# FluxML/Flux3D.jl

Measured on AMD Instinct MI355X. Metric: chamfer_point_pairs_per_sec, higher is better.
Workload: dtype f32

## Files before the change

flux3d.jl_amd/csrc/chamfer.hip:

```cpp
#include <atomic>
#include <cmath>
#include <cstdlib>
#include <mutex>

#include "fx3d_common.h"

using namespace fx3d;

#ifdef FX3D_PROBE
__device__ unsigned long long g_probe[4096 * 16];
#define FX3D_PROBE_MARK(k)                                                                   \
    do {                                                                                     \
        if (threadIdx.x == 0 && blockIdx.x < 4096) {                                         \
            g_probe[blockIdx.x * 16 + (k)] = __builtin_readcyclecounter();                   \
            if ((k) == 0) g_probe[blockIdx.x * 16 + 13] = wall_clock64();                    \
            if ((k) == 12) g_probe[blockIdx.x * 16 + 14] = wall_clock64();                   \
        }                                                                                    \
    } while (0)
__device__ unsigned long long g_probe2[256 * 16];
#define FX3D_PROBE_MARK2(k) do { if (threadIdx.x == 0 && blockIdx.x < 256) g_probe2[blockIdx.x * 16 + (k)] = __builtin_readcyclecounter(); } while (0)
__device__ unsigned long long g_probe3[16 * 16 * 8];
#define FX3D_PROBE_MARKW(k) do { if ((threadIdx.x & 63) == 0 && blockIdx.x < 16) g_probe3[(blockIdx.x * 16 + (threadIdx.x >> 6)) * 8 + (k)] = __builtin_readcyclecounter(); } while (0)
#else
#define FX3D_PROBE_MARK(k) do { } while (0)
// ... 311 lines not shown
__device__ __forceinline__ float vmin(float a, float b) {
    float r;
    asm("v_min_f32 %0, %1, %2" : "=v"(r) : "v"(a), "v"(b));
    return r;
}

__device__ __forceinline__ void split2h(float v, _Float16 &h, _Float16 &l) {
    h = (_Float16)v;
    l = (_Float16)(v - (float)h);
}

constexpr float kBetaC = 0x1.1p-18f;
constexpr float kBandB1 = 1.0f + 18.0f * kBetaC + 0x1p-20f;
constexpr float kBandA = 22.3f * kBetaC + 0x1p-19f;
__device__ __forceinline__ void make_pieces(float cx, float cy, float cz, h8 &p0, h8 &p1) {
    _Float16 hx, lx, hy, ly, hz, lz, n1, n2, n3;
    split2h(cx, hx, lx); split2h(cy, hy, ly); split2h(cz, hz, lz);
    const float n0 = ((cx * cx) + (cy * cy)) + (cz * cz);
    const float n = n0 + kBetaC * n0;
    n1 = (_Float16)n;
    const float r1 = n - (float)n1;
    n2 = (_Float16)r1;
    n3 = (_Float16)(r1 - (float)n2);
    const _Float16 z = (_Float16)0.0f;
    p0 = h8{hx, hx, lx, hy, hy, ly, hz, hz};
    p1 = h8{lz, n1, n2, n3, lx, ly, lz, z};
}

template <bool WANT_IDX, bool SPLITFUSE = false, bool PRUNE = false>
__global__ __launch_bounds__(kHThreads, 4) void nn1_f16_kernel(Nn1Params p) {
    extern __shared__ __attribute__((aligned(16))) float lds[];
    __shared__ __attribute__((aligned(16))) float red[4 * 4 * (kHThreads / 64) + 16];
    __shared__ int nfar[2];
    __shared__ unsigned short farlist[kHFarCap];
    constexpr int QB = (kHThreads / 64) * 32;

    const int L = blockIdx.x;
    const int per_cloud = p.tiles * p.nsplit;
    const bool by_xcd = 2 * p.B >= 8;
    const int slot = by_xcd ? L >> 3 : L;
    const int c = by_xcd ? (slot / per_cloud) * 8 + (L & 7) : slot / per_cloud;
    const int tile = (slot % per_cloud) / p.nsplit;
    const int split = (slot % per_cloud) % p.nsplit;
    if (c >= 2 * p.B) return;
    const int dir = c >= p.B ? 1 : 0;
    const int b = dir ? c - p.B : c;
    const int NQ = dir ? p.M : p.N;
    const int NC = dir ? p.N : p.M;
    if (tile >= (dir ? p.tiles_y : p.tiles_x)) return;
    if ((long long)split * p.chunk >= NC) return;
    const int ctail = (p.tail > 0 && p.nsplit == 1 && NC > p.chunk && NC - p.chunk <= p.tail) ? NC - p.chunk : 0;
    const int NCm = NC - ctail;
    const float *__restrict__ qb = (dir ? p.y : p.x) + (size_t)b * NQ * 3;
    const float *__restrict__ cb = (dir ? p.x : p.y) + (size_t)b * NC * 3;
    int32_t *idx_out = dir ? p.idx_y : p.idx_x;
    float *dmin_out = dir ? p.dmin_y : p.dmin_x;

    const int tid = threadIdx.x, lane = tid & 63;
    const int wv = __builtin_amdgcn_readfirstlane(tid >> 6);
    const int jq = lane & 31, hh = lane >> 5;
    const int CH = p.chunk;
    const int tpb = dir ? p.tpb_y : p.tpb;
    h8 *imgp = reinterpret_cast<h8 *>(lds);
    float4 *imgf = reinterpret_cast<float4 *>(lds);
    unsigned long long *wres = reinterpret_cast<unsigned long long *>(lds + 8 * (CH + 64));
    unsigned short *witems = reinterpret_cast<unsigned short *>(wres + (kHThreads / 64) * 32);
    float *wq = reinterpret_cast<float *>(witems + (kHThreads / 64) * kHItemCap);
    unsigned long long *qres = wres + wv * 32;
    unsigned short *items = witems + wv * kHItemCap;
    float *qtab = wq + wv * 96;
    const bool vec = (reinterpret_cast<uintptr_t>(cb) & 15) == 0;
    const bool one_shot = NCm <= CH;
    if (tid == 0) { nfar[0] = 0; nfar[1] = 0; }
    float qpre[3];
    {
        const int q0i = (tile * tpb) * QB + wv * 32 + jq;
        const int qc0 = q0i < NQ ? q0i : NQ - 1;
#pragma unroll
        for (int d = 0; d < 3; ++d) qpre[d] = qb[(size_t)qc0 * 3 + d];
    }
    if constexpr (PRUNE) {
        unsigned int *zc = reinterpret_cast<unsigned int *>(wres);
        for (int i = tid; i < 1040 + 16 * 256; i += kHThreads) zc[i] = 0u;
        int *gb = reinterpret_cast<int *>(wq + (kHThreads / 64) * 96) + 64 * 8;
        for (int i = tid; i < kHGroupsMax * 8; i += kHThreads) gb[i] = (i & 4) ? (int)0x80000000 : 0x7fffffff;
    }
    FX3D_PROBE_MARK(0);

    const bool own_chunk_only = p.nsplit > 1 && (long long)split * CH + (long long)p.nsplit * CH >= NCm;
    const int s_lo = own_chunk_only ? split * CH : 0;
    const int SN = own_chunk_only ? (NCm - s_lo < CH ? NCm - s_lo : CH) : NC;
    const float *__restrict__ sb = cb + (size_t)s_lo * 3;
    const bool parked = one_shot || own_chunk_only;
    float mu[3], cinf = 0.0f, varmax = 0.0f;
    float bxlo[3] = {0.f, 0.f, 0.f}, bxhi[3] = {0.f, 0.f, 0.f};
    bool allfin = true;
    {
        float mn[3] = {INFINITY, INFINITY, INFINITY}, mx[3] = {-INFINITY, -INFINITY, -INFINITY}, sm3[3] = {0.f, 0.f, 0.f};
        float sqt = 0.0f;
        const float pil[3] = {sb[0], sb[1], sb[2]};
        const int nsweep = (SN + kHThreads - 1) / kHThreads;
        for (int i0 = 0; i0 < nsweep; i0 += 4) {
            P3 v[4];
#pragma unroll
            for (int e = 0; e < 4; ++e) {
                const int pt = (i0 + e) * kHThreads + tid;
                v[e] = *reinterpret_cast<const P3 *>(sb + (size_t)(pt < SN ? pt : SN - 1) * 3);
            }
#pragma unroll
            for (int e = 0; e < 4; ++e) {
                const int pt = (i0 + e) * kHThreads + tid;
                mn[0] = fminf(mn[0], v[e].x); mx[0] = fmaxf(mx[0], v[e].x);
                mn[1] = fminf(mn[1], v[e].y); mx[1] = fmaxf(mx[1], v[e].y);
                mn[2] = fminf(mn[2], v[e].z); mx[2] = fmaxf(mx[2], v[e].z);
                if (pt < SN) {
                    sm3[0] = sm3[0] + v[e].x; sm3[1] = sm3[1] + v[e].y; sm3[2] = sm3[2] + v[e].z;
                    if (parked) imgf[((pt >> 5) * 2) * 32 + (pt & 31)] = float4{v[e].x, v[e].y, v[e].z, 0.0f};
                }
                if (((i0 + e) & 3) == (wv & 3) && pt < SN) {
                    sqt = __builtin_fmaf(v[e].x - pil[0], v[e].x - pil[0], sqt); sqt = __builtin_fmaf(v[e].y - pil[1], v[e].y - pil[1], sqt);
                    sqt = __builtin_fmaf(v[e].z - pil[2], v[e].z - pil[2], sqt);
                }
            }
        }
        FX3D_PROBE_MARK(5);
        {
            float4 lo4, hi4, st4;
            lo4.x = wave_min_l63(mn[0]); lo4.y = wave_min_l63(mn[1]); lo4.z = wave_min_l63(mn[2]); lo4.w = 0.0f;
            hi4.x = wave_max_l63(mx[0]); hi4.y = wave_max_l63(mx[1]); hi4.z = wave_max_l63(mx[2]); hi4.w = 0.0f;
            st4.x = wave_sum_l63(sm3[0]); st4.y = wave_sum_l63(sm3[1]); st4.z = wave_sum_l63(sm3[2]); st4.w = wave_sum_l63(sqt);
            if (lane == 63) {
                float4 *r4 = reinterpret_cast<float4 *>(red);
                r4[wv * 4] = lo4; r4[wv * 4 + 1] = hi4; r4[wv * 4 + 2] = st4;
            }
        }
        FX3D_PROBE_MARK(9);
        __syncthreads();
        FX3D_PROBE_MARK(10);
        static_assert(kHThreads / 64 == 16, "the cross-wave reduction below: one wave's row of 16 lanes, one lane per wave");
        if (wv == 0) {
            const float4 *r4 = reinterpret_cast<const float4 *>(red);
            const int w = lane & 15;
            float4 lo4 = r4[w * 4], hi4 = r4[w * 4 + 1], st4 = r4[w * 4 + 2];
#define NN1_ROW_MIN(v) v = fkey_inv(row_mm_key<false>(fkey(v)));
#define NN1_ROW_MAX(v) v = fkey_inv(row_mm_key<true>(fkey(v)));
#define NN1_ROW_SUM(v) v = v + dpp_mov<0xB1>(v); v = v + dpp_mov<0x4E>(v); v = v + dpp_mov<0x141>(v); v = v + dpp_mov<0x140>(v);
            NN1_ROW_MIN(lo4.x) NN1_ROW_MIN(lo4.y) NN1_ROW_MIN(lo4.z)
            NN1_ROW_MAX(hi4.x) NN1_ROW_MAX(hi4.y) NN1_ROW_MAX(hi4.z)
            NN1_ROW_SUM(st4.x) NN1_ROW_SUM(st4.y) NN1_ROW_SUM(st4.z) NN1_ROW_SUM(st4.w)
#undef NN1_ROW_MIN
#undef NN1_ROW_MAX
#undef NN1_ROW_SUM
            const float lo3[3] = {lo4.x, lo4.y, lo4.z}, hi3[3] = {hi4.x, hi4.y, hi4.z}, st3[3] = {st4.x, st4.y, st4.z};
            float m3[3], ci = 0.0f, vm = st4.w / fmaxf(0.25f * (float)SN, 1.0f);
            bool fin = true;
#pragma unroll
            for (int d = 0; d < 3; ++d) {
                const float lo = lo3[d], hi = hi3[d], st = st3[d];
                m3[d] = fminf(fmaxf(st / (float)SN, lo), hi);
                const float off = st / (float)SN - pil[d];
                vm = vm - off * off;
                ci = fmaxf(ci, fmaxf(hi - m3[d], m3[d] - lo));
                fin = fin && fabsf(st) < INFINITY;
            }
            if (lane == 0) {
                float4 *o4 = reinterpret_cast<float4 *>(red) + 4 * (kHThreads / 64);
                o4[0] = float4{m3[0], m3[1], m3[2], ci * 1.000001f};
                o4[1] = float4{vm, fin ? 1.0f : 0.0f, 0.0f, 0.0f};
                if (PRUNE) { o4[2] = float4{lo3[0], lo3[1], lo3[2], 0.0f}; o4[3] = float4{hi3[0], hi3[1], hi3[2], 0.0f}; }
            }
        }
        __syncthreads();
        {
            const float4 *o4 = reinterpret_cast<const float4 *>(red) + 4 * (kHThreads / 64);
            const float4 a = o4[0], b2 = o4[1];
            mu[0] = a.x; mu[1] = a.y; mu[2] = a.z; cinf = a.w;
            varmax = b2.x; allfin = b2.y != 0.0f;
            if (PRUNE) {
                const float4 l4 = o4[2], h4 = o4[3];
                bxlo[0] = l4.x; bxlo[1] = l4.y; bxlo[2] = l4.z; bxhi[0] = h4.x; bxhi[1] = h4.y; bxhi[2] = h4.z;
            }
        }
    }
    float rng = cinf;
    if (allfin && cinf < 1.0e16f && 3.0f * cinf * cinf > kRobustGate * varmax) {
        const float4 r = robust_range3<kHThreads, false>(sb, SN, parked, imgf, red, mu[0], mu[1], mu[2], cinf);
        mu[0] = r.x; mu[1] = r.y; mu[2] = r.z; rng = r.w;
    }
    const bool sane = allfin && cinf < 1.0e16f;
    float sc = 1.0f;
    if (sane && rng > 1.0e-30f) {
        int e;
        (void)frexpf(rng, &e);
        sc = ldexpf(1.0f, 7 - e);
    }
    auto uni = [](float v) { return __builtin_bit_cast(float, __builtin_amdgcn_readfirstlane(__builtin_bit_cast(int, v))); };
    mu[0] = uni(mu[0]); mu[1] = uni(mu[1]); mu[2] = uni(mu[2]); sc = uni(sc); rng = uni(rng); cinf = uni(cinf);
    const bool has_far = sane && rng < cinf;
    int fslot = 0;
    auto pieces = [&](float x, float y, float z, int pt, h8 &p0, h8 &p1) {
        const float sx = (x - mu[0]) * sc, sy = (y - mu[1]) * sc, sz = (z - mu[2]) * sc;
        if (!has_far) { make_pieces(sx, sy, sz, p0, p1); return; }
        const bool far = !(fmaxf(fmaxf(fabsf(sx), fabsf(sy)), fabsf(sz)) < 128.0f);
        make_pieces(far ? 0.f : sx, far ? 0.f : sy, far ? 0.f : sz, p0, p1);
        if (far) {
            p1[7] = (_Float16)kPadF16;
            const int f = atomicAdd(&nfar[fslot], 1);
            if (f < kHFarCap) farlist[f] = (unsigned short)pt;
        }
    };

    [[maybe_unused]] float4 *cs = nullptr, *qsw = nullptr;
    [[maybe_unused]] bool sorted_c = false;
    [[maybe_unused]] int qwlen = 0;
    [[maybe_unused]] float4 *boxes = nullptr;
    if constexpr (PRUNE) {
        cs = p.pscr + (size_t)blockIdx.x * p.pscr_stride;
        qsw = cs + kHChunkMax;
        boxes = reinterpret_cast<float4 *>(wq + (kHThreads / 64) * 96);
        unsigned int *ccnt = reinterpret_cast<unsigned int *>(wres);
        unsigned int *qtot = ccnt + 520;
        unsigned int *qwh = qtot + 520;
        const bool last_t = tile == (dir ? p.tiles_y : p.tiles_x) - 1;
        const int qw0 = tile * tpb * QB;
        const int qw1 = last_t || qw0 + tpb * QB > NQ ? NQ : qw0 + tpb * QB;
        qwlen = qw1 - qw0;
        const int cnt = NCm;
        const bool do_sort = sane && cnt >= 512;
        const bool sorted_q = do_sort && NQ <= 4 * kHThreads;
        P3 qv[4];
        if (sorted_q) {
#pragma unroll
            for (int e = 0; e < 4; ++e) {
                const int qp = 256 * wv + 64 * e + lane;
                qv[e] = *reinterpret_cast<const P3 *>(qb + (size_t)(qp < NQ ? qp : NQ - 1) * 3);
            }
        }
        FX3D_PROBE_MARK2(0);
        int *gbox = reinterpret_cast<int *>(boxes + 64 * 2);
        auto group_box = [&](int wrow, float x, float y, float z) {
            int *g = gbox + (wrow >> 5) * 8;
            atomicMin(g + 0, fkey((x - mu[0]) * sc)); atomicMin(g + 1, fkey((y - mu[1]) * sc)); atomicMin(g + 2, fkey((z - mu[2]) * sc));
            atomicMax(g + 4, fkey((x - mu[0]) * sc)); atomicMax(g + 5, fkey((y - mu[1]) * sc)); atomicMax(g + 6, fkey((z - mu[2]) * sc));
        };
        if (do_sort) {
            float4 cv[4];
#pragma unroll
            for (int e = 0; e < 4; ++e) {
                const int pt = e * kHThreads + tid;
                cv[e] = float4{0.f, 0.f, 0.f, 0.f};
                if (pt < cnt) cv[e] = imgf[((pt >> 5) * 2) * 32 + (pt & 31)];
            }
            FX3D_PROBE_MARK2(1);
            float inv[3], off[3], cfl[3], cfh[3];
#pragma unroll
            for (int d = 0; d < 3; ++d) {
                const float fr = has_far ? 0.125f * rng : 128.0f / sc;
                const float flo = fmaxf(bxlo[d], mu[d] - fr), fhi = fminf(bxhi[d], mu[d] + fr);
                inv[d] = fhi > flo ? 8.0f / (fhi - flo) : 0.0f;
                off[d] = -flo * inv[d];
                cfl[d] = flo; cfh[d] = fhi;
            }
            auto cell = [&](float x, float y, float z) -> unsigned int {
                const unsigned int ux = (unsigned int)(int)fminf(fmaxf(__builtin_fmaf(x, inv[0], off[0]), 0.0f), 7.0f);
                const unsigned int uy = (unsigned int)(int)fminf(fmaxf(__builtin_fmaf(y, inv[1], off[1]), 0.0f), 7.0f);
                const unsigned int uz = (unsigned int)(int)fminf(fmaxf(__builtin_fmaf(z, inv[2], off[2]), 0.0f), 7.0f);
                return ux | (uy << 3) | (uz << 6);
            };

            unsigned int ccr[4], qcr[4];
            auto count_cells = [&](bool valid, unsigned int t, auto &&add) -> unsigned int {
                unsigned int rank = 0u;
                bool mine = valid;
                const unsigned int tn = (unsigned int)__builtin_amdgcn_update_dpp((int)~t, (int)t, 0x111, 0xF, 0xF, false);
                if (__builtin_popcountll(__ballot(valid && t == tn)) >= 8) {
                    unsigned long long rem = __ballot(valid);
                    for (int it = 0; it < 12 && rem; ++it) {
                        const unsigned int t0 = (unsigned int)__builtin_amdgcn_readlane((int)t, __builtin_ctzll(rem));
                        const unsigned long long grp = __ballot(mine && t == t0);
                        rem &= ~grp;
                        if (__builtin_popcountll(grp) < 4) continue;
                        unsigned int base = 0u;
                        if ((int)lane == __builtin_ctzll(grp)) base = add(t0, (unsigned int)__builtin_popcountll(grp));
                        base = (unsigned int)__builtin_amdgcn_readlane((int)base, __builtin_ctzll(grp));
                        if (mine && t == t0) {
                            rank = base + __builtin_amdgcn_mbcnt_hi((unsigned int)(grp >> 32), __builtin_amdgcn_mbcnt_lo((unsigned int)grp, 0u));
                            mine = false;
                        }
                    }
                }
                if (mine) rank = add(t, 1u);
                return rank;
            };
#pragma unroll
            for (int e = 0; e < 4; ++e) {
                const int pt = e * kHThreads + tid;
                const unsigned int t = pt < cnt ? cell(cv[e].x, cv[e].y, cv[e].z) : 0u;
                ccr[e] = (t << 16) | count_cells(pt < cnt, t, [&](unsigned int c, unsigned int n) { return atomicAdd(&ccnt[c], n); });
            }
            int *qbb = reinterpret_cast<int *>(boxes + 64 * 2 + kHGroupsMax * 2 - 2);
            if (sorted_q) {
                int kl[3] = {0x7fffffff, 0x7fffffff, 0x7fffffff}, kh[3] = {(int)0x80000000, (int)0x80000000, (int)0x80000000};
#pragma unroll
                for (int e = 0; e < 4; ++e) {
                    const int qp = 256 * wv + 64 * e + lane;
                    if (qp < NQ) {
                        const int k3[3] = {fkey(qv[e].x), fkey(qv[e].y), fkey(qv[e].z)};
#pragma unroll
                        for (int d = 0; d < 3; ++d) { kl[d] = kl[d] < k3[d] ? kl[d] : k3[d]; kh[d] = kh[d] > k3[d] ? kh[d] : k3[d]; }
                    }
                }
#pragma unroll
                for (int d = 0; d < 3; ++d) {
                    int a = row_mm_key<false>(kl[d]), b2 = row_mm_key<true>(kh[d]);
                    a = imm<false>(a, dpp_keepi<0x142, 0xA>(a)); a = imm<false>(a, dpp_keepi<0x143, 0xC>(a));
                    b2 = imm<true>(b2, dpp_keepi<0x142, 0xA>(b2)); b2 = imm<true>(b2, dpp_keepi<0x143, 0xC>(b2));
                    if (lane == 63) { atomicMin(qbb + d, a); atomicMax(qbb + 4 + d, b2); }
                }
            }
            FX3D_PROBE_MARK2(2);
            __syncthreads();
            FX3D_PROBE_MARK2(3);
            float qinv[3] = {0.f, 0.f, 0.f}, qoff[3] = {0.f, 0.f, 0.f};
            if (sorted_q) {
                const float ext = fmaxf(fmaxf(cfh[0] - cfl[0], cfh[1] - cfl[1]), cfh[2] - cfl[2]);
#pragma unroll
                for (int d = 0; d < 3; ++d) {
                    const float ql = fkey_inv(qbb[d]), qh = fkey_inv(qbb[4 + d]);
                    const float grow = qh - ql > 4.0f * ext ? 0.25f * ext : ext;
                    const float lo = fmaxf(ql, cfl[d] - grow), hi = fminf(qh, cfh[d] + grow);
                    qinv[d] = hi > lo && hi - lo < INFINITY ? 8.0f / (hi - lo) : 0.0f;
                    qoff[d] = qinv[d] != 0.0f ? -lo * qinv[d] : 0.0f;
                }
            }
            auto qcell = [&](float x, float y, float z) -> unsigned int {
                const unsigned int ux = (unsigned int)(int)fminf(fmaxf(__builtin_fmaf(x, qinv[0], qoff[0]), 0.0f), 7.0f);
                const unsigned int uy = (unsigned int)(int)fminf(fmaxf(__builtin_fmaf(y, qinv[1], qoff[1]), 0.0f), 7.0f);
                const unsigned int uz = (unsigned int)(int)fminf(fmaxf(__builtin_fmaf(z, qinv[2], qoff[2]), 0.0f), 7.0f);
                return ux | (uy << 3) | (uz << 6);
            };
            auto curve_scan = [&](unsigned int *a) {
                unsigned int tc[8];
                {
                    const uint4 h = *reinterpret_cast<const uint4 *>(kHilbertCell + 8 * lane);
                    tc[0] = h.x & 0xffffu; tc[1] = h.x >> 16; tc[2] = h.y & 0xffffu; tc[3] = h.y >> 16;
                    tc[4] = h.z & 0xffffu; tc[5] = h.z >> 16; tc[6] = h.w & 0xffffu; tc[7] = h.w >> 16;
                }
                unsigned int c8[8], tot = 0u;
#pragma unroll
                for (int k = 0; k < 8; ++k) { c8[k] = a[tc[k]]; tot += c8[k]; }
                unsigned int inc = tot;
#pragma unroll
                for (int o = 1; o < 64; o <<= 1) {
                    const unsigned int v = __shfl_up(inc, o, 64);
                    if (lane >= o) inc += v;
                }
                unsigned int run = inc - tot;
#pragma unroll
                for (int k = 0; k < 8; ++k) { a[tc[k]] = run; run += c8[k]; }
            };
            if (wv == 0) curve_scan(ccnt);
            if (sorted_q) {
#pragma unroll
                for (int e = 0; e < 4; ++e) {
                    const int qp = 256 * wv + 64 * e + lane;
                    const unsigned int t = qp < NQ ? qcell(qv[e].x, qv[e].y, qv[e].z) : 0u;
                    qcr[e] = (t << 16) | count_cells(qp < NQ, t, [&](unsigned int c, unsigned int n) {
                                 const unsigned int sh = 16u * (c & 1u);
                                 const unsigned int old = atomicAdd(&qwh[wv * 256 + (c >> 1)], n << sh);
                                 atomicAdd(&qtot[c], n);
                                 return (old >> sh) & 0xffffu;
                             });
                }
            }
            FX3D_PROBE_MARK2(4);
            __syncthreads();
            FX3D_PROBE_MARK2(5);
#pragma unroll
            for (int e = 0; e < 4; ++e) {
                const int pt = e * kHThreads + tid;
                if (pt < cnt) {
                    const int pos = (int)(ccnt[ccr[e] >> 16] + (ccr[e] & 0xffffu));
                    imgf[((pos >> 5) * 2) * 32 + (pos & 31)] = float4{cv[e].x, cv[e].y, cv[e].z, __builtin_bit_cast(float, pt)};
                }
            }
            sorted_c = true;
            if (sorted_q) {
                if (wv == 1) {
                    curve_scan(qtot);
                } else if (wv >= 2 && wv < 6) {
                    const int w2 = tid - 128;
                    unsigned int run = 0u;
#pragma unroll
                    for (int w = 0; w < 16; ++w) {
                        const unsigned int v = qwh[w * 256 + w2];
                        qwh[w * 256 + w2] = run;
                        run += v;
                    }
                }
            }
            FX3D_PROBE_MARK2(6);
            __syncthreads();
            FX3D_PROBE_MARK2(7);
            if (sorted_q) {
#pragma unroll
                for (int e = 0; e < 4; ++e) {
                    const int qp = 256 * wv + 64 * e + lane;
                    if (qp < NQ) {
                        const unsigned int t = qcr[e] >> 16;
                        const int rank = (int)(qtot[t] + ((qwh[wv * 256 + (t >> 1)] >> (16u * (t & 1u))) & 0xffffu) + (qcr[e] & 0xffffu));
                        if (rank >= qw0 && rank < qw1) {
                            qsw[rank - qw0] = float4{qv[e].x, qv[e].y, qv[e].z, __builtin_bit_cast(float, qp)};
                            group_box(rank - qw0, qv[e].x, qv[e].y, qv[e].z);
                        }
                    }
                }
            }
        }
        if (!sorted_q) {
            for (int q0 = qw0 + wv * 64; q0 < qw1; q0 += kHThreads) {
                const int qp = q0 + lane;
                const P3 r = *reinterpret_cast<const P3 *>(qb + (size_t)(qp < qw1 ? qp : qw1 - 1) * 3);
                if (qp < qw1) qsw[qp - qw0] = float4{r.x, r.y, r.z, __builtin_bit_cast(float, qp)};
                const int kx = fkey((r.x - mu[0]) * sc), ky = fkey((r.y - mu[1]) * sc), kz = fkey((r.z - mu[2]) * sc);
                const int lx = row_mm_key<false>(kx), ly = row_mm_key<false>(ky), lz = row_mm_key<false>(kz);
                const int hx = row_mm_key<true>(kx), hy = row_mm_key<true>(ky), hz = row_mm_key<true>(kz);
                if ((lane & 15) == 0 && qp < qw1) {
                    int *g = gbox + ((qp - qw0) >> 5) * 8;
                    atomicMin(g + 0, lx); atomicMin(g + 1, ly); atomicMin(g + 2, lz);
                    atomicMax(g + 4, hx); atomicMax(g + 5, hy); atomicMax(g + 6, hz);
                }
            }
        }
        FX3D_PROBE_MARK2(8);
    }
    FX3D_PROBE_MARK(1);

    const float cm2 = 3.0f * (fminf(cinf * sc, 128.0f) * fminf(cinf * sc, 128.0f));
    float qr[3], da = 0.0f;
    float da_far = 0.0f;
    [[maybe_unused]] float dpr = INFINITY;
    bool qfin = true;
    int qi = 0;
    bool qok = true;
    h8 bq;
    double acc = 0.0;

    const int jfirst = split * CH, jstep = p.nsplit * CH;
    for (int j0 = jfirst; j0 < NCm; j0 += jstep) {
        const int cnt = (NCm - j0) < CH ? (NCm - j0) : CH;
        const int cnt_pad = (cnt + 32 * kHLT - 1) / (32 * kHLT) * (32 * kHLT);
        if (j0 > jfirst) __syncthreads();
        if constexpr (PRUNE) {
            for (int tl = tid >> 4; tl * 64 < cnt_pad + 64; tl += kHThreads / 16) {
                float4 r4[4];
#pragma unroll
                for (int k = 0; k < 4; ++k) {
                    const int pt = tl * 64 + k * 16 + (tid & 15);
                    r4[k] = float4{0.f, 0.f, 0.f, 0.f};
                    if (pt < cnt) r4[k] = imgf[((pt >> 5) * 2) * 32 + (pt & 31)];
                }
                float lo3[3] = {INFINITY, INFINITY, INFINITY}, hi3[3] = {-INFINITY, -INFINITY, -INFINITY};
#pragma unroll
                for (int k = 0; k < 4; ++k) {
                    const int pt = tl * 64 + k * 16 + (tid & 15), i0 = ((pt >> 5) * 2) * 32 + (pt & 31);
                    h8 p0, p1;
                    if (pt < cnt) {
                        pieces(r4[k].x, r4[k].y, r4[k].z, pt, p0, p1);
                        const int id = sorted_c ? __builtin_bit_cast(int, r4[k].w) : j0 + pt;
                        cs[pt] = float4{r4[k].x, r4[k].y, r4[k].z, __builtin_bit_cast(float, id)};
                        const float b3[3] = {(r4[k].x - mu[0]) * sc, (r4[k].y - mu[1]) * sc, (r4[k].z - mu[2]) * sc};
#pragma unroll
                        for (int d = 0; d < 3; ++d) { lo3[d] = vmin(lo3[d], b3[d]); hi3[d] = -vmin(-hi3[d], -b3[d]); }
                    } else {
                        make_pieces(0.f, 0.f, 0.f, p0, p1);
                        p1[7] = (_Float16)kPadF16;
                    }
                    imgp[i0] = p0;
                    imgp[i0 + 32] = p1;
                }
                float bl[3], bh[3];
#pragma unroll
                for (int d = 0; d < 3; ++d) { bl[d] = fkey_inv(row_mm_key<false>(fkey(lo3[d]))); bh[d] = fkey_inv(row_mm_key<true>(fkey(hi3[d]))); }
                if ((tid & 15) == 0 && tl < 64) {
                    boxes[tl * 2] = float4{bl[0], bl[1], bl[2], 0.0f};
                    boxes[tl * 2 + 1] = float4{bh[0], bh[1], bh[2], 0.0f};
                }
            }
        } else
        for (int pt = tid; pt < cnt_pad + 64; pt += kHThreads) {
            const int i0 = ((pt >> 5) * 2) * 32 + (pt & 31);
            h8 p0, p1;
            if (pt < cnt) {
                if (parked) {
                    const float4 r = imgf[i0];
                    pieces(r.x, r.y, r.z, pt, p0, p1);
                } else {
                    const P3 r = *reinterpret_cast<const P3 *>(cb + (size_t)(j0 + pt) * 3);
                    pieces(r.x, r.y, r.z, pt, p0, p1);
                }
            } else {
                make_pieces(0.f, 0.f, 0.f, p0, p1);
                p1[7] = (_Float16)kPadF16;
            }
            imgp[i0] = p0;
            imgp[i0 + 32] = p1;
        }
        __syncthreads();
        FX3D_PROBE_MARK(j0 == jfirst ? 2 : 6);
        FX3D_PROBE_MARKW(0);

        const int nf = nfar[fslot];
        if (tid == 0) nfar[fslot ^ 1] = 0;
        fslot ^= 1;
        const bool far_ok = nf <= kHFarCap;
        const bool last_tile = tile == (dir ? p.tiles_y : p.tiles_x) - 1;
        for (int tp = 0; tp < tpb || (last_tile && one_shot); ++tp) {
            if ((tile * tpb + tp) * QB >= NQ) break;
            if constexpr (PRUNE) {
                if (tp * QB + wv * 32 >= qwlen) continue;
            }
            if (j0 == jfirst) {
                qi = (tile * tpb + tp) * QB + wv * 32 + jq;
                if constexpr (PRUNE) {
                    const int wpos = tp * QB + wv * 32 + jq;
                    const float4 q4 = qsw[wpos < qwlen ? wpos : qwlen - 1];
                    qr[0] = q4.x; qr[1] = q4.y; qr[2] = q4.z;
                    qi = wpos < qwlen ? __builtin_bit_cast(int, q4.w) : NQ;
                } else if (tp == 0) {
#pragma unroll
                    for (int d = 0; d < 3; ++d) qr[d] = qpre[d];
                } else {
                    const int qc1 = qi < NQ ? qi : NQ - 1;
#pragma unroll
                    for (int d = 0; d < 3; ++d) qr[d] = qb[(size_t)qc1 * 3 + d];
                }
                float m0 = -2.0f * ((qr[0] - mu[0]) * sc), m1 = -2.0f * ((qr[1] - mu[1]) * sc), m2 = -2.0f * ((qr[2] - mu[2]) * sc);
                float S = (fabsf(m0) + fabsf(m1)) + fabsf(m2);
                float sq = 1.0f, fl_s = 0.0f;
                if (S >= 3.0e4f && S < 0x1p28f) {
                    int e;
                    (void)frexpf(S, &e);
                    sq = ldexpf(1.0f, 14 - e);
                    m0 *= sq; m1 *= sq; m2 *= sq; S *= sq;
                    fl_s = 0x1p-15f;
                }
                qok = S < 3.0e4f;
                qfin = fabsf(qr[0]) + fabsf(qr[1]) + fabsf(qr[2]) < INFINITY;
                const float qn = 0.25f * ((m0 * m0 + m1 * m1) + m2 * m2) / sq;
                da = kBandA * qn + 0x1p-24f * (S + 4.0f) + fl_s;
                {
                    const float c2 = sq * cm2;
                    da_far = 2.1f * kBetaC * c2 + 2.0f * kBetaC * sqrtf(qn * c2) + 0x1p-19f * qn + 0x1p-24f * (S + 4.0f) + fl_s;
                }
                if constexpr (PRUNE) {
                    dpr = qok && sq == 1.0f ? qn + 2.0f * kBetaC * (cm2 + qn) + 0x1p-23f * (S + 4.0f) : INFINITY;
                }
                _Float16 hx, lx, hy, ly, hz, lz;
                split2h(qok ? m0 : 0.f, hx, lx); split2h(qok ? m1 : 0.f, hy, ly); split2h(qok ? m2 : 0.f, hz, lz);
                const _Float16 one = (_Float16)sq, pad = (_Float16)kPadF16;
                bq = hh == 0 ? h8{hx, lx, hx, hy, ly, hy, hz, lz} : h8{hz, one, one, one, lx, ly, lz, pad};
                if (hh == 0) {
                    qres[jq] = ~0ull;
                    qtab[jq * 3 + 0] = qr[0]; qtab[jq * 3 + 1] = qr[1]; qtab[jq * 3 + 2] = qr[2];
                }
            }

            float tm = INFINITY, fk[kHFifo];
#pragma unroll
            for (int s = 0; s < kHFifo; ++s) fk[s] = INFINITY;
            const unsigned int keymask = ~((1u << kHIdBits) - 1u);

            static_assert(kHLT == 2, "the rotation below is written for lane tiles of two blocks");
            const int nblk = cnt_pad / 32;
            f32x16 zero;
#pragma unroll
            for (int r = 0; r < 16; ++r) zero[r] = 0.0f;
#define NN1_FOLD(ACC, FIRST)                                                                                         \
            {                                                                                                        \
                const float t0 = min3f(ACC[0], ACC[1], ACC[2]), t1 = min3f(ACC[3], ACC[4], ACC[5]);                  \
                const float t2 = min3f(ACC[6], ACC[7], ACC[8]), t3 = min3f(ACC[9], ACC[10], ACC[11]);                \
                const float t4 = min3f(ACC[12], ACC[13], ACC[14]);                                                   \
                const float t5 = min3f(t0, t1, t2), t6 = min3f(t3, t4, ACC[15]);                                     \
                tm = (FIRST) ? vmin(t5, t6) : min3f(tm, t5, t6);       \
            }
#define NN1_TRACK_ID(LT)                                                                                             \
            {                                                                                                        \
                float key;                                                                                           \
                asm("v_and_or_b32 %0, %1, %2, %3" : "=v"(key) : "v"(tm), "v"(keymask), "s"(LT));                     \
                _Pragma("unroll") for (int s_ = kHFifo - 1; s_ > 0; --s_) fk[s_] = __builtin_amdgcn_fmed3f(fk[s_ - 1], fk[s_], key);    \
                fk[0] = vmin(fk[0], key);                                                                            \
            }
#define NN1_TRACK() { NN1_TRACK_ID(lt) ++lt; }
#define NN1_CLOSE(ACC, ODD, LT)                                                                                      \
            if constexpr (kHBlkTrack) { NN1_FOLD(ACC, true) NN1_TRACK_ID(2 * (LT) + (ODD)) }                           \
            else { NN1_FOLD(ACC, !(ODD)) if (ODD) NN1_TRACK_ID(LT) }
#define NN1_STEP(ISSUE, FOLD, ODD, OFF)                                                                              \
            __builtin_amdgcn_s_setprio(0);                                                                           \
            ISSUE = __builtin_amdgcn_mfma_f32_32x32x16_f16(an, bq, zero, 0, 0, 0);                                   \
            an = pa[(OFF) * 64];                                                                                     \
            __builtin_amdgcn_s_setprio(1);                                                                           \
            NN1_CLOSE(FOLD, ODD, lt)                                                                                 \
            if (ODD) ++lt;
            if constexpr (!PRUNE) {
            const h8 *pa = imgp + hh * 32 + jq;
            f32x16 acc0, acc1, acc2;
            h8 an = pa[0];
            acc0 = __builtin_amdgcn_mfma_f32_32x32x16_f16(an, bq, zero, 0, 0, 0); an = pa[1 * 64];
            acc1 = __builtin_amdgcn_mfma_f32_32x32x16_f16(an, bq, zero, 0, 0, 0); an = pa[2 * 64];
            pa += 3 * 64;
            int lt = 0;
            int nb = 2;
            for (; nb + 6 <= nblk; nb += 6) {
                NN1_STEP(acc2, acc0, 0, 0) NN1_STEP(acc0, acc1, 1, 1) NN1_STEP(acc1, acc2, 0, 2)
                NN1_STEP(acc2, acc0, 1, 3) NN1_STEP(acc0, acc1, 0, 4) NN1_STEP(acc1, acc2, 1, 5)
                pa += 6 * 64;
            }
            if (nblk - nb == 4) {
                NN1_STEP(acc2, acc0, 0, 0) NN1_STEP(acc0, acc1, 1, 1) NN1_STEP(acc1, acc2, 0, 2) NN1_STEP(acc2, acc0, 1, 3)
                NN1_CLOSE(acc1, 0, lt) NN1_CLOSE(acc2, 1, lt)
            } else if (nblk - nb == 2) {
                NN1_STEP(acc2, acc0, 0, 0) NN1_STEP(acc0, acc1, 1, 1)
                NN1_CLOSE(acc2, 0, lt) NN1_CLOSE(acc0, 1, lt)
            } else {
                NN1_CLOSE(acc0, 0, lt) NN1_CLOSE(acc1, 1, lt)
            }
            } else {
            const int nltp = nblk / kHLT;
            float bd = INFINITY;
            {
                const int4 *gq = reinterpret_cast<const int4 *>(boxes + 64 * 2) + (tp * (kHThreads / 64) + wv) * 2;
                const int4 gl = gq[0], gh = gq[1];
                const float qlx = fkey_inv(gl.x), qly = fkey_inv(gl.y), qlz = fkey_inv(gl.z);
                const float qhx = fkey_inv(gh.x), qhy = fkey_inv(gh.y), qhz = fkey_inv(gh.z);
                if (lane < nltp) {
                    const float4 lo = boxes[lane * 2], hi = boxes[lane * 2 + 1];
                    const float gx = fmaxf(fmaxf(lo.x - qhx, qlx - hi.x), 0.0f), gy = fmaxf(fmaxf(lo.y - qhy, qly - hi.y), 0.0f);
                    const float gz = fmaxf(fmaxf(lo.z - qhz, qlz - hi.z), 0.0f);
                    bd = (gx * gx + gy * gy) + gz * gz;
                }
            }
            const unsigned long long all_lt = nltp >= 64 ? ~0ull : (1ull << nltp) - 1ull;
            unsigned long long todo = all_lt, done = 0ull;
            if (sorted_c) {
                todo = __ballot(bd == 0.0f);
                if (!todo) {
                    const float bmin = wave_min_f(bd);
                    todo = bmin < INFINITY ? __ballot(bd == bmin) : all_lt;
                }
            }
            const h8 *pbase = imgp + hh * 32 + jq;
            for (int phase = 0; phase < 2; ++phase) {
                if (phase == 1) {
                    if (done == all_lt) break;
                    const float kb = fk[0];
                    const float bb = __builtin_fmaf(fabsf(kb), kKeyUp, kb);
                    const float dj = fminf(bb, __shfl_xor(bb, 32, 64)) + dpr;
                    const float ucut = wave_max_f(__builtin_fmaf(dj, 1.0f + 0x1p-9f, 0x1p-8f));
                    const bool keep = !(bd > ucut) || !(dj == dj);
                    todo = (__ballot(!(dj == dj)) ? all_lt : __ballot(keep)) & all_lt & ~done;
                    if (!todo) break;
                }
                done |= todo;
                unsigned long long mk = todo;
                int nrem = __builtin_popcountll(mk) - 1;
#define NN1_NEXT(T) { T = nltp; if (mk) { T = __builtin_ctzll(mk); mk &= mk - 1ull; } }
                int ta, tb;
                NN1_NEXT(ta) NN1_NEXT(tb)
                f32x16 acc0, acc1, acc2;
                const h8 *pn = pbase + ta * (kHLT * 64);
                h8 an = pn[0];
                acc0 = __builtin_amdgcn_mfma_f32_32x32x16_f16(an, bq, zero, 0, 0, 0); an = pn[64];
                pn = pbase + tb * (kHLT * 64);
                acc1 = __builtin_amdgcn_mfma_f32_32x32x16_f16(an, bq, zero, 0, 0, 0); an = pn[0];
#define NN1_PSTEP(ISSUE, FOLD, ODD, LT, NEXT)                                                                         \
                __builtin_amdgcn_s_setprio(0);                                                                       \
                ISSUE = __builtin_amdgcn_mfma_f32_32x32x16_f16(an, bq, zero, 0, 0, 0);                               \
                an = NEXT;                                                                                           \
                __builtin_amdgcn_s_setprio(1);                                                                       \
                NN1_CLOSE(FOLD, ODD, LT)
                while (nrem >= 3) {
                    int tc, td, te;
                    NN1_NEXT(tc) NN1_NEXT(td) NN1_NEXT(te)
                    nrem -= 3;
                    const h8 *pc = pbase + tc * (kHLT * 64), *pd = pbase + td * (kHLT * 64);
                    NN1_PSTEP(acc2, acc0, 0, ta, pn[64])
                    NN1_PSTEP(acc0, acc1, 1, ta, pc[0])
                    pn = pbase + te * (kHLT * 64);
                    NN1_PSTEP(acc1, acc2, 0, tb, pc[64])
                    NN1_PSTEP(acc2, acc0, 1, tb, pd[0])
                    NN1_PSTEP(acc0, acc1, 0, tc, pd[64])
                    NN1_PSTEP(acc1, acc2, 1, tc, pn[0])
                    ta = td; tb = te;
                }
                if (nrem == 2) {
                    int tc;
                    NN1_NEXT(tc)
                    const h8 *pc = pbase + tc * (kHLT * 64);
                    NN1_PSTEP(acc2, acc0, 0, ta, pn[64])
                    NN1_PSTEP(acc0, acc1, 1, ta, pc[0])
                    NN1_PSTEP(acc1, acc2, 0, tb, pc[64])
                    NN1_PSTEP(acc2, acc0, 1, tb, pc[64])
                    NN1_CLOSE(acc1, 0, tc) NN1_CLOSE(acc2, 1, tc)
                } else if (nrem == 1) {
                    NN1_PSTEP(acc2, acc0, 0, ta, pn[64])
                    NN1_PSTEP(acc0, acc1, 1, ta, pn[64])
                    NN1_CLOSE(acc2, 0, tb) NN1_CLOSE(acc0, 1, tb)
                } else {
                    NN1_CLOSE(acc0, 0, ta) NN1_CLOSE(acc1, 1, ta)
                }
#undef NN1_PSTEP
#undef NN1_NEXT
                __builtin_amdgcn_s_setprio(0);
#ifdef FX3D_PROBE_COUNT
                if ((threadIdx.x & 63) == 0) atomicAdd(&g_probe[4095 * 16 + 6 + phase], (unsigned long long)__builtin_popcountll(todo));
#endif
            }
// ... 699 lines not shown
        return pl;
    }
    if (pl.variant == 0) {
        const int per_block = kThreads * R;
        pl.tiles_x = (N + per_block - 1) / per_block;
        pl.tiles_y = (M + per_block - 1) / per_block;
        pl.tiles = pl.tiles_x > pl.tiles_y ? pl.tiles_x : pl.tiles_y;
        int chunk = (maxc0 + kTile - 1) / kTile * kTile;
        if (chunk > kChunkMax) chunk = kChunkMax;
        pl.chunk = chunk;
        pl.lds_bytes = (size_t)chunk * (D <= 3 ? D : 0) * sizeof(float);
        pl.grid = clouds8 * 8 * pl.tiles;
        return pl;
    }
    const int cmax = kHChunkMax, gran = 32 * kHLT;
    const int ncu = device_cus();
    int maxc = maxc0, b_chunk = 0, b_tpb = 1, b_split = 1;
    auto search = [&](int mc) {
        maxc = mc;
        const int cminc = (maxc + cmax - 1) / cmax;
        double best = 1e30;
        b_chunk = (maxc + gran - 1) / gran * gran < cmax ? (maxc + gran - 1) / gran * gran : cmax; b_tpb = 1; b_split = 1;
        for (int nch = cminc; nch <= cminc * 8 && nch <= 64; ++nch) {
            int ch = ((maxc + nch - 1) / nch + gran - 1) / gran * gran;
            if (ch > cmax) continue;
            const int anch = (maxc + ch - 1) / ch;
            for (int split = 0; split < 2; ++split) {
                if (split && (!allow_split || anch == 1 || opt(OPT_NN1_NOSPLIT))) continue;
                for (int tpb = 1; tpb <= 8; tpb *= 2) {
                    if (!split && anch > 1 && tpb > 1) continue;
                    const long long tiles = ((long long)maxc + 512 * tpb - 1) / (512 * tpb);
                    const long long blocks = 2ll * B * tiles * (split ? anch : 1);
                    const double per_chunk = 5.0 * ch / 4096.0 + 0.5 + tpb * (9.7 * ch / 4096.0 + 0.8);
                    const double t_block = 2.8 * maxc / 4096.0 + (split ? 1 : anch) * per_chunk;
                    const double rounds = (double)((blocks + ncu - 1) / ncu);
                    const double t = rounds * t_block + (split ? 8.0 : 0.0);
                    if (t < best - 1e-9) { best = t; b_chunk = ch; b_tpb = tpb; b_split = split ? anch : 1; }
                }
            }
        }
    };
    pl.tail = 0;
    if (maxc0 > cmax && maxc0 - cmax <= kHTail) {
        search(cmax);
        if (b_split == 1 && b_chunk == cmax) pl.tail = kHTail;
    }
    if (!pl.tail) search(maxc0);
    pl.chunk = b_chunk;
    pl.tpb = pl.tpb_y = b_tpb;
    pl.nsplit = b_split;
    pl.lds_bytes = (size_t)pl.chunk * 8 * sizeof(float) + kHScratchBytes;
    if (N != M && b_split == 1 && maxc <= b_chunk) {
        double bt = 1e30;
        for (int ta = 1; ta <= 8; ta *= 2)
            for (int tb = 1; tb <= 8; tb *= 2) {
                const double blk_a = 2.8 * M / 4096.0 + 5.0 * M / 4096.0 + 0.5 + ta * (9.7 * M / 4096.0 + 0.8);
                const double blk_b = 2.8 * N / 4096.0 + 5.0 * N / 4096.0 + 0.5 + tb * (9.7 * N / 4096.0 + 0.8);
                const double na = (double)B * ((N + 512 * ta - 1) / (512 * ta)), nb = (double)B * ((M + 512 * tb - 1) / (512 * tb));
                const double thr = (na * blk_a + nb * blk_b) / (double)ncu;
                double t = blk_a > blk_b ? blk_a : blk_b;
                t = t > thr ? t : thr;
                const long long tmax = (N + 512 * ta - 1) / (512 * ta) > (M + 512 * tb - 1) / (512 * tb) ? (N + 512 * ta - 1) / (512 * ta) : (M + 512 * tb - 1) / (512 * tb);
                t += 1.0 * (double)((2ll * B * tmax + ncu - 1) / ncu - 1);
                if (t < bt - 1e-9) { bt = t; pl.tpb = ta; pl.tpb_y = tb; }
            }
    }
    const bool fold = b_split == 1 && maxc <= b_chunk;
    auto ntiles = [&](int nq, int tpb) {
        const int per = 512 * tpb;
        int t = (nq + per - 1) / per;
        if (fold && t > 1 && nq - (t - 1) * per <= kHTail) --t;
        return t;
    };
    pl.tiles_x = ntiles(N, pl.tpb);
    pl.tiles_y = ntiles(M, pl.tpb_y);
    pl.tiles = pl.tiles_x > pl.tiles_y ? pl.tiles_x : pl.tiles_y;
    pl.grid = clouds8 * 8 * pl.tiles * pl.nsplit;
    if (2 * B < 8) pl.grid = 2 * B * pl.tiles * pl.nsplit;
    return pl;
}

size_t partials_count(const Plan &pl, int B) { return (size_t)2 * B * pl.tiles; }

constexpr size_t kHBoxBytes = 64 * 2 * sizeof(float4) + kHGroupsMax * 32;
int prune_rows_per_block(const Plan &pl, int N, int M, int D) {
    const int maxc = N > M ? N : M;
    if (D != 3 || pl.variant != 3 || pl.nsplit != 1 || pl.tail != 0 || maxc > pl.chunk || maxc < 1024 || !opt(OPT_NN1_PRUNE)) return 0;
    if ((pl.tpb > pl.tpb_y ? pl.tpb : pl.tpb_y) * 16 + 2 > kHGroupsMax - 1) return 0;
    if ((pl.tpb < pl.tpb_y ? pl.tpb : pl.tpb_y) < 2) return 0;
    return kHChunkMax + (pl.tpb > pl.tpb_y ? pl.tpb : pl.tpb_y) * 512 + kHTail;
}
size_t prune_scratch_bytes(const Plan &pl, int N, int M, int D) {
    return (size_t)prune_rows_per_block(pl, N, M, D) * pl.grid * sizeof(float4);
}

template <int DIM, bool WANT_IDX>
fx3d_status launch_small(const Nn1Params &p, const Plan &pl, hipStream_t st) {
    if (pl.variant == 4) {
        if (DIM == 3) {
            const bool small = (p.N > p.M ? p.N : p.M) <= kTySl * kTyG;
            if (pl.R == 2 && small) hipLaunchKernelGGL((nn1_tiny_kernel<2, 1, WANT_IDX>), dim3(pl.grid), dim3(kTyThreads), 0, st, p);
            else if (pl.R == 2) hipLaunchKernelGGL((nn1_tiny_kernel<2, 4, WANT_IDX>), dim3(pl.grid), dim3(kTyThreads), 0, st, p);
            else if (small) hipLaunchKernelGGL((nn1_tiny_kernel<1, 1, WANT_IDX>), dim3(pl.grid), dim3(kTyThreads), 0, st, p);
            else hipLaunchKernelGGL((nn1_tiny_kernel<1, 4, WANT_IDX>), dim3(pl.grid), dim3(kTyThreads), 0, st, p);
        }
        FX3D_LAUNCH_CHECK();
        return FX3D_OK;
    }
    if (pl.variant == 3) {
        if (DIM == 3) {
            const void *kfn = p.pscr ? reinterpret_cast<const void *>(&nn1_f16_kernel<WANT_IDX, false, true>)
                              : p.fuse_split ? reinterpret_cast<const void *>(&nn1_f16_kernel<WANT_IDX, true>)
                                             : reinterpret_cast<const void *>(&nn1_f16_kernel<WANT_IDX, false>);
            const fx3d_status arc = ensure_dynamic_lds(kfn, (int)(kHChunkMax * 32 + kHScratchBytes + (p.pscr ? kHBoxBytes : 0)), "nn1_f16_kernel");
            if (arc != FX3D_OK) return arc;
            if (p.pscr) hipLaunchKernelGGL((nn1_f16_kernel<WANT_IDX, false, true>), dim3(pl.grid), dim3(kHThreads), pl.lds_bytes + kHBoxBytes, st, p);
            else if (p.fuse_split) hipLaunchKernelGGL((nn1_f16_kernel<WANT_IDX, true>), dim3(pl.grid), dim3(kHThreads), pl.lds_bytes, st, p);
            else hipLaunchKernelGGL((nn1_f16_kernel<WANT_IDX, false>), dim3(pl.grid), dim3(kHThreads), pl.lds_bytes, st, p);
        }
        FX3D_LAUNCH_CHECK();
        return FX3D_OK;
    }
    switch (pl.R) {
        case 4:
            hipLaunchKernelGGL((nn1_small_d_kernel<DIM, 4, WANT_IDX>), dim3(pl.grid), dim3(kThreads), pl.lds_bytes, st, p);
            break;
        case 2:
            hipLaunchKernelGGL((nn1_small_d_kernel<DIM, 2, WANT_IDX>), dim3(pl.grid), dim3(kThreads), pl.lds_bytes, st, p);
            break;
        default:
            hipLaunchKernelGGL((nn1_small_d_kernel<DIM, 1, WANT_IDX>), dim3(pl.grid), dim3(kThreads), pl.lds_bytes, st, p);
            break;
    }
    FX3D_LAUNCH_CHECK();
    return FX3D_OK;
}

fx3d_status check_shapes(const char *fn, const void *x, int N, const void *y, int M, int B, int D) {
    FX3D_REQUIRE(x && y, "%s: null input pointer", fn);
    FX3D_REQUIRE(N > 0 && M > 0 && B > 0 && D > 0, "%s: empty input (N=%d M=%d B=%d D=%d)", fn, N, M, B, D);
    FX3D_REQUIRE((long long)B * 2 * (((long long)(N > M ? N : M) + 255) / 256) < (1ll << 30),
                 "%s: problem too large for one launch", fn);
    return FX3D_OK;
}

constexpr long long kSplitFuseMax = 255;
struct Fused {
    unsigned int *ticket;
    unsigned int nvalid;
    double *sums_out;
    float *loss_out;
    float w1, w2;
    long long Bg;
};

fx3d_status run_nn1(const float *x, int N, const float *y, int M, int B, int D, int32_t *idx_x,
                    int32_t *idx_y, float *dmin_x, float *dmin_y, double *partials,
                    const Plan &pl, hipStream_t st, const Fused *fu = nullptr,
                    unsigned long long *gres = nullptr, int qstride = 0, float4 *pscr = nullptr) {
    Nn1Params p{};
    p.pscr = pscr;
    p.pscr_stride = pscr ? prune_rows_per_block(pl, N, M, D) : 0;
    if (!p.pscr_stride) p.pscr = nullptr;
    p.nsplit = gres ? pl.nsplit : 1;
    p.gres = gres;
    p.qstride = qstride;
    p.fuse_split = gres && fu && fu->ticket ? 1 : 0;
// ... 263 lines not shown
```

Baseline: 14590 billion.

## Compute per-wave query bounding boxes with readlane instead of shared-memory atomics

Removes the per-group query bounding-box accumulation, which used LDS atomicMin/atomicMax during query staging, along with its shared-memory table and initialisation. Each wave now derives its query box at use time. It reduces per-lane keys with row_mm_key on sign-flipped keys and combines them with readlanes. The query staging loop becomes a plain copy, and pad-row writing moves to the last wave instead of an extra loop iteration. This cuts atomic traffic and LDS footprint, but the box must match the wave's actual query set and the hh-based sign trick must be correct.

```diff
diff --git a/flux3d.jl_amd/csrc/chamfer.hip b/flux3d.jl_amd/csrc/chamfer.hip
--- a/flux3d.jl_amd/csrc/chamfer.hip
+++ b/flux3d.jl_amd/csrc/chamfer.hip
@@ -417,8 +417,8 @@
     if constexpr (PRUNE) {
         unsigned int *zc = reinterpret_cast<unsigned int *>(wres);
         for (int i = tid; i < 1040 + 16 * 256; i += kHThreads) zc[i] = 0u;
-        int *gb = reinterpret_cast<int *>(wq + (kHThreads / 64) * 96) + 64 * 8;
-        for (int i = tid; i < kHGroupsMax * 8; i += kHThreads) gb[i] = (i & 4) ? (int)0x80000000 : 0x7fffffff;
+        int *qbb0 = reinterpret_cast<int *>(wq + (kHThreads / 64) * 96) + 64 * 8;
+        if (tid < 8) qbb0[tid] = (tid & 4) ? (int)0x80000000 : 0x7fffffff;
     }
     FX3D_PROBE_MARK(0);
 
@@ -572,12 +572,6 @@
             }
         }
         FX3D_PROBE_MARK2(0);
-        int *gbox = reinterpret_cast<int *>(boxes + 64 * 2);
-        auto group_box = [&](int wrow, float x, float y, float z) {
-            int *g = gbox + (wrow >> 5) * 8;
-            atomicMin(g + 0, fkey((x - mu[0]) * sc)); atomicMin(g + 1, fkey((y - mu[1]) * sc)); atomicMin(g + 2, fkey((z - mu[2]) * sc));
-            atomicMax(g + 4, fkey((x - mu[0]) * sc)); atomicMax(g + 5, fkey((y - mu[1]) * sc)); atomicMax(g + 6, fkey((z - mu[2]) * sc));
-        };
         if (do_sort) {
             float4 cv[4];
 #pragma unroll
@@ -633,7 +627,7 @@
                 const unsigned int t = pt < cnt ? cell(cv[e].x, cv[e].y, cv[e].z) : 0u;
                 ccr[e] = (t << 16) | count_cells(pt < cnt, t, [&](unsigned int c, unsigned int n) { return atomicAdd(&ccnt[c], n); });
             }
-            int *qbb = reinterpret_cast<int *>(boxes + 64 * 2 + kHGroupsMax * 2 - 2);
+            int *qbb = reinterpret_cast<int *>(boxes + 64 * 2);
             if (sorted_q) {
                 int kl[3] = {0x7fffffff, 0x7fffffff, 0x7fffffff}, kh[3] = {(int)0x80000000, (int)0x80000000, (int)0x80000000};
 #pragma unroll
@@ -744,27 +738,15 @@
                     if (qp < NQ) {
                         const unsigned int t = qcr[e] >> 16;
                         const int rank = (int)(qtot[t] + ((qwh[wv * 256 + (t >> 1)] >> (16u * (t & 1u))) & 0xffffu) + (qcr[e] & 0xffffu));
-                        if (rank >= qw0 && rank < qw1) {
-                            qsw[rank - qw0] = float4{qv[e].x, qv[e].y, qv[e].z, __builtin_bit_cast(float, qp)};
-                            group_box(rank - qw0, qv[e].x, qv[e].y, qv[e].z);
-                        }
+                        if (rank >= qw0 && rank < qw1) qsw[rank - qw0] = float4{qv[e].x, qv[e].y, qv[e].z, __builtin_bit_cast(float, qp)};
                     }
                 }
             }
         }
         if (!sorted_q) {
-            for (int q0 = qw0 + wv * 64; q0 < qw1; q0 += kHThreads) {
-                const int qp = q0 + lane;
-                const P3 r = *reinterpret_cast<const P3 *>(qb + (size_t)(qp < qw1 ? qp : qw1 - 1) * 3);
-                if (qp < qw1) qsw[qp - qw0] = float4{r.x, r.y, r.z, __builtin_bit_cast(float, qp)};
-                const int kx = fkey((r.x - mu[0]) * sc), ky = fkey((r.y - mu[1]) * sc), kz = fkey((r.z - mu[2]) * sc);
-                const int lx = row_mm_key<false>(kx), ly = row_mm_key<false>(ky), lz = row_mm_key<false>(kz);
-                const int hx = row_mm_key<true>(kx), hy = row_mm_key<true>(ky), hz = row_mm_key<true>(kz);
-                if ((lane & 15) == 0 && qp < qw1) {
-                    int *g = gbox + ((qp - qw0) >> 5) * 8;
-                    atomicMin(g + 0, lx); atomicMin(g + 1, ly); atomicMin(g + 2, lz);
-                    atomicMax(g + 4, hx); atomicMax(g + 5, hy); atomicMax(g + 6, hz);
-                }
+            for (int qp = qw0 + tid; qp < qw1; qp += kHThreads) {
+                const P3 r = *reinterpret_cast<const P3 *>(qb + (size_t)qp * 3);
+                qsw[qp - qw0] = float4{r.x, r.y, r.z, __builtin_bit_cast(float, qp)};
             }
         }
         FX3D_PROBE_MARK2(8);
@@ -775,6 +757,7 @@
     float qr[3], da = 0.0f;
     float da_far = 0.0f;
     [[maybe_unused]] float dpr = INFINITY;
+    [[maybe_unused]] int gk[3];
     bool qfin = true;
     int qi = 0;
     bool qok = true;
@@ -787,7 +770,15 @@
         const int cnt_pad = (cnt + 32 * kHLT - 1) / (32 * kHLT) * (32 * kHLT);
         if (j0 > jfirst) __syncthreads();
         if constexpr (PRUNE) {
-            for (int tl = tid >> 4; tl * 64 < cnt_pad + 64; tl += kHThreads / 16) {
+            if (tid >= kHThreads - 64) {
+                const int pt = cnt_pad + (tid & 63), i0 = ((pt >> 5) * 2) * 32 + (pt & 31);
+                h8 p0, p1;
+                make_pieces(0.f, 0.f, 0.f, p0, p1);
+                p1[7] = (_Float16)kPadF16;
+                imgp[i0] = p0;
+                imgp[i0 + 32] = p1;
+            }
+            for (int tl = tid >> 4; tl * 64 < cnt_pad; tl += kHThreads / 16) {
                 float4 r4[4];
 #pragma unroll
                 for (int k = 0; k < 4; ++k) {
@@ -898,6 +889,11 @@
                 if (hh == 0) {
                     qres[jq] = ~0ull;
                     qtab[jq * 3 + 0] = qr[0]; qtab[jq * 3 + 1] = qr[1]; qtab[jq * 3 + 2] = qr[2];
+                }
+                if constexpr (PRUNE) {
+                    const int hm = -hh;
+#pragma unroll
+                    for (int d = 0; d < 3; ++d) gk[d] = row_mm_key<false>(fkey((qr[d] - mu[d]) * sc) ^ hm);
                 }
             }
 
@@ -964,10 +960,15 @@
             const int nltp = nblk / kHLT;
             float bd = INFINITY;
             {
-                const int4 *gq = reinterpret_cast<const int4 *>(boxes + 64 * 2) + (tp * (kHThreads / 64) + wv) * 2;
-                const int4 gl = gq[0], gh = gq[1];
-                const float qlx = fkey_inv(gl.x), qly = fkey_inv(gl.y), qlz = fkey_inv(gl.z);
-                const float qhx = fkey_inv(gh.x), qhy = fkey_inv(gh.y), qhz = fkey_inv(gh.z);
+                float ql3[3], qh3[3];
+#pragma unroll
+                for (int d = 0; d < 3; ++d) {
+                    const int l0 = __builtin_amdgcn_readlane(gk[d], 0), l1 = __builtin_amdgcn_readlane(gk[d], 16);
+                    const int h0 = __builtin_amdgcn_readlane(gk[d], 32), h1 = __builtin_amdgcn_readlane(gk[d], 48);
+                    ql3[d] = fkey_inv(l0 < l1 ? l0 : l1);
+                    qh3[d] = fkey_inv(~(h0 < h1 ? h0 : h1));
+                }
+                const float qlx = ql3[0], qly = ql3[1], qlz = ql3[2], qhx = qh3[0], qhy = qh3[1], qhz = qh3[2];
                 if (lane < nltp) {
                     const float4 lo = boxes[lane * 2], hi = boxes[lane * 2 + 1];
                     const float gx = fmaxf(fmaxf(lo.x - qhx, qlx - hi.x), 0.0f), gy = fmaxf(fmaxf(lo.y - qhy, qly - hi.y), 0.0f);
@@ -1833,7 +1834,7 @@
 
 size_t partials_count(const Plan &pl, int B) { return (size_t)2 * B * pl.tiles; }
 
-constexpr size_t kHBoxBytes = 64 * 2 * sizeof(float4) + kHGroupsMax * 32;
+constexpr size_t kHBoxBytes = 64 * 2 * sizeof(float4) + 32;
 int prune_rows_per_block(const Plan &pl, int N, int M, int D) {
     const int maxc = N > M ? N : M;
     if (D != 3 || pl.variant != 3 || pl.nsplit != 1 || pl.tail != 0 || maxc > pl.chunk || maxc < 1024 || !opt(OPT_NN1_PRUNE)) return 0;
```

Result: no change. 14680 billion (median of 6 runs) (+0.6%).
